# SiftScience/kafka-assigner

Hardware: NVIDIA H100
Metric: partition-replica assignments/sec (higher is better)
Workload: dtype int32

## Files before the change

kafka_assigner_b200/csrc/kassign.cu:

```cuda
#include "kassign_stage.cuh"
#include "kassign_order.cuh"
#include "kassign_json.cuh"
#include "kassign_score.cuh"
#include "kassign_waves.cuh"
#include "kassign_waves_json.cuh"

#include <algorithm>
#include <climits>
#include <cmath>
#include <cstdio>
#include <cstdlib>
#include <cstring>
#include <map>
#include <new>
#include <string>
#include <unordered_map>
#include <vector>

#include "../../include/kassign.h"

namespace {

constexpr int KA_SM_COUNT_FALLBACK = 132;
constexpr size_t KA_SMEM_BUDGET = 200 * 1024;
constexpr uint32_t KA_LUT_SMEM_MAX_RANGE = 32768;
constexpr uint32_t KA_LUT_GLOBAL_MAX_RANGE = 1u << 25;

struct DevBuf {
    void* p = nullptr;
    size_t cap = 0;
    cudaError_t reserve(size_t bytes) {
        if (bytes <= cap) return cudaSuccess;
        if (p) cudaFree(p);
        p = nullptr;
        cap = 0;
        size_t want = bytes + bytes / 8 + 256;
        cudaError_t e = cudaMalloc(&p, want);
        if (e == cudaSuccess) cap = want;
        return e;
    }
    void release() {
        if (p) cudaFree(p);
        p = nullptr;
        cap = 0;
    }
    template <typename T> T* as() const { return reinterpret_cast<T*>(p); }
};

constexpr int KA_MAX_BLOCKS = 8;
constexpr int KA_MAX_CHAIN_BLOCKS = 8;
constexpr int KA_MAX_CHAIN_EVENTS = 64;
constexpr int KA_MAX_JSON_FRAGS = 256;
constexpr int KA_MAX_CANDIDATES = 128;
static_assert(KA_MAX_CANDIDATES <= KA_JSON_MAX_SEGS, "a fleet's documents are built in one segmented JSON pass");
constexpr int64_t KA_JSON_FRAG_ROWS = 1 << 18;

struct HostPinned {
    int err_topic;
    int spin_flag;
    int4 tstatus;
};

struct Plan {
    int a_blob_bytes;
    int a_warps, a_load_bytes, a_slab_bytes, a_cnt_bytes, a_load_kind;
    int a_levels;
    int lv_owner_bytes, lv_last_bytes, lv_p_bytes;
    size_t a_smem;
    int rec_kind, rec_bytes;
    int b_gctr;
    int b_ring_log2;
    int b_threads;
    size_t b_smem;
};

struct StageDesc {
    int topic_base = 0, T = 0;
    int64_t Q = 0;
    const int32_t* d_hash = nullptr;
    const int64_t* d_part_off = nullptr;
    const int64_t* d_rep_off = nullptr;
    int P = 0, RF = 0;
    const int32_t* d_cur = nullptr;
    int desired_rf = -1, S = 1, Pmax = 0;
// ... 19 lines not shown
    }
};

}

struct ka_ctx {
    int device = 0;
    int sm_count = KA_SM_COUNT_FALLBACK;
    cudaStream_t stream = nullptr;
    cudaStream_t aux = nullptr;
    cudaStream_t sb1 = nullptr;
    cudaStream_t sj = nullptr;
    KaBrokers br{};
    std::vector<int32_t> broker_id;
    DevBuf d_blob, d_glut, d_broker_id, d_ctr8;
    std::unordered_map<int32_t, std::vector<int32_t>> parked;
    int64_t launches = 0;
    DevBuf d_hash, d_part_off, d_rep_off, d_cur, d_out, d_out_len;
    RunScratch run;
    DevBuf d_json, d_names, d_name_off, d_part_id, d_json_rowlen, d_json_blocksum, d_json_state;
    DevBuf d_json_seg;
    DevBuf d_batch_tab, d_batch_ctr;
    RunScratch batch_run;
    DevBuf d_score_w, d_score_sum, d_score_brk, d_score_off;
    DevBuf d_wv_nrecv, d_wv_wave, d_wv_tmp, d_wv_rec, d_wv_cnt, d_wv_state, d_wv_log, d_wv_sum, d_wv_meta;
    DevBuf d_wv_send, d_wv_slog, d_wv_ssum;
    DevBuf d_wv_perm, d_wv_hist, d_wv_doc;
    DevBuf d_wv_part, d_wv_jump;
    DevBuf d_wv_back, d_wv_bscr;
    HostPinned* h_pin = nullptr;
    unsigned long long* h_frag = nullptr;
    cudaEvent_t ev[6] = {};
    cudaEvent_t ev_pipe[KA_MAX_BLOCKS][5] = {};
    cudaEvent_t ev_chain[KA_MAX_CHAIN_EVENTS][4] = {};
    cudaEvent_t ev_in = nullptr, ev_stage[KA_MAX_BLOCKS] = {}, ev_chain_in = nullptr, ev_b1[KA_MAX_CHAIN_EVENTS] = {};
    cudaEvent_t ev_json_in[KA_MAX_JSON_FRAGS] = {}, ev_json_scan[KA_MAX_JSON_FRAGS] = {}, ev_out_done = nullptr;
    bool timing = false;
    float last_ms[8] = {};
    bool ev_valid = false;
    int last_stages = 1;
    int chain_used = 0;
    bool slot_timed[2] = {false, false};
    int32_t order_plan[8] = {};
    int32_t stage_plan[8] = {};
    bool staged = false;
    StageDesc staged_block;
    int topic_base = 0;
    bool last_was_staged = false;
    cudaStream_t last_stream = nullptr;
    bool pending_status = false;
    ka_status last{};
};

namespace {

#define KA_CUDA(call)                                                                              \
    do {                                                                                           \
        cudaError_t _e = (call);                                                                   \
        if (_e != cudaSuccess) {                                                                   \
            std::fprintf(stderr, "[kassign] CUDA error %s at %s:%d: %s\n", cudaGetErrorName(_e), __FILE__, __LINE__, \
                         cudaGetErrorString(_e));                                                  \
            return KA_ERR_CUDA;                                                                    \
        }                                                                                          \
    } while (0)

int set_status(ka_status* st, int code, int topic = -1, int part = -1, int a = 0, int b = 0) {
    if (st) {
        st->code = code;
        st->topic_index = topic;
        st->partition = part;
        st->a = a;
        st->b = b;
    }
    return code;
}

int failed(ka_status* st, int rc) {
    if (st && st->code != rc) set_status(st, rc);
    return rc;
}

inline size_t align16(size_t v) { return (v + 15) & ~size_t(15); }

template <typename F>
void for_each_event(ka_ctx* c, F f) {
    const struct { cudaEvent_t* e; size_t n; bool timed; } pools[] = {
        {c->ev, sizeof(c->ev) / sizeof(cudaEvent_t), true},
        {&c->ev_pipe[0][0], sizeof(c->ev_pipe) / sizeof(cudaEvent_t), true},
        {&c->ev_chain[0][0], sizeof(c->ev_chain) / sizeof(cudaEvent_t), true},
        {&c->ev_in, 1, false},
        {c->ev_stage, KA_MAX_BLOCKS, false},
        {&c->ev_chain_in, 1, false},
        {c->ev_b1, KA_MAX_CHAIN_EVENTS, false},
        {c->ev_json_in, KA_MAX_JSON_FRAGS, false},
        {c->ev_json_scan, KA_MAX_JSON_FRAGS, false},
        {&c->ev_out_done, 1, false},
    };
    for (const auto& p : pools)
        for (size_t i = 0; i < p.n; ++i) f(p.e[i], p.timed);
}

int park_counters(ka_ctx* c) {
    if (c->br.N == 0 || !c->d_ctr8.p) return KA_OK;
    std::vector<int32_t> h((size_t)c->br.N * KA_MAX_SLOTS);
    KA_CUDA(cudaMemcpy(h.data(), c->d_ctr8.p, h.size() * 4, cudaMemcpyDeviceToHost));
    for (int i = 0; i < c->br.N; ++i) {
        const int32_t* row = h.data() + (size_t)i * KA_MAX_SLOTS;
        bool nz = false;
        for (int r = 0; r < KA_MAX_SLOTS; ++r) nz |= row[r] != 0;
        if (nz) c->parked[c->broker_id[i]] = std::vector<int32_t>(row, row + KA_MAX_SLOTS);
        else c->parked.erase(c->broker_id[i]);
    }
    return KA_OK;
}

int check_brokers(int N, const int32_t* broker_id, const int32_t* broker_rack) {
    if (N < 0 || (N > 0 && (!broker_id || !broker_rack))) return KA_ERR_BAD_ARG;
    if (N > 65535) return KA_ERR_LIMIT;
    for (int i = 0; i < N; ++i) {
        if (i > 0 && broker_id[i] <= broker_id[i - 1]) return KA_ERR_BAD_ARG;
        if (broker_rack[i] < 0 || broker_rack[i] >= 65535) return KA_ERR_BAD_ARG;
    }
    return KA_OK;
}

struct BrokerTable {
// ... 254 lines not shown
    return p;
}

int enq_stage(ka_ctx* c, cudaStream_t s, const StageDesc& d, cudaEvent_t a_done) {
    const Plan& pl = d.pl;
    RunScratch& r = c->run;
    if (d.T > 0) {
        KaSolveParams p = stage_params(d);
        p.br = c->br;
        p.out.rec = r.rec.as<unsigned char>() + (size_t)d.q0 * pl.rec_bytes;
        p.out.perm = pl.a_levels ? r.perm.as<uint16_t>() + d.q0 : nullptr;
        p.out.ntl = pl.a_levels ? r.ntl.as<int32_t>() + d.topic_base : nullptr;
        p.out.lend = pl.a_levels ? r.lend.as<uint32_t>() + d.q0 : nullptr;
        p.out.tstatus = r.tstatus.as<int4>();
        p.out.err_topic = r.flags.as<unsigned>();
        const int rc = launch_stage_plan<false>(c, s, p, pl, d.T, 0, 1 << c->br.lut_mode);
        if (rc != KA_OK) return rc;
    }
    if (c->timing) KA_CUDA(cudaEventRecord(a_done, s));
    if (pl.a_levels && d.T > 0) {
        int32_t* ntl = r.ntl.as<int32_t>() + d.topic_base;
        int32_t* loff = r.loff.as<int32_t>() + d.topic_base + d.blk;
        ka_level_scan_kernel<<<1, 1024, 0, s>>>(ntl, d.T, loff);
        KA_CUDA(cudaGetLastError());
        ka_level_fill_kernel<<<(d.T + 7) / 8, 256, 0, s>>>(ntl, loff, r.lend.as<uint32_t>() + d.q0, d.d_part_off, d.P, d.T, d.T, d.Q,
                                                            r.lvl_end.as<uint32_t>() + d.q0);
        KA_CUDA(cudaGetLastError());
        c->launches += 2;
    }
    return KA_OK;
}

template <int KIND, int MAXNT, bool CAND, bool GCTR, bool SINGLE, bool WARP1, bool FULL>
cudaError_t launch_order_t(cudaStream_t s, const KaOrderParams& o, const Plan& pl, int ncand) {
    auto kern = ka_order_levels_kernel<KIND, GCTR, MAXNT, SINGLE, WARP1, FULL, CAND>;
    cudaError_t e = allow_smem(kern, pl.b_smem);
    if (e != cudaSuccess) return e;
    kern<<<CAND ? ncand : 1, pl.b_threads, pl.b_smem, s>>>(o);
    return cudaGetLastError();
}

template <int KIND, int MAXNT, bool CAND = false>
cudaError_t launch_order(cudaStream_t s, const KaOrderParams& o, const Plan& pl, int* sel, int ncand = 0) {
    if constexpr (KIND > 1) {
        *sel = pl.b_gctr ? 4 : 0;
        return pl.b_gctr ? launch_order_t<KIND, MAXNT, false, true, false, false, false>(s, o, pl, ncand)
                         : launch_order_t<KIND, MAXNT, false, false, false, false, false>(s, o, pl, ncand);
    } else {
        const bool warp1 = pl.b_threads == 32;
        const bool single = !warp1 && o.uniform_width != 0 && o.uniform_width <= (uint32_t)pl.b_threads;
        const bool full = single && o.uniform_width == (uint32_t)pl.b_threads;
        *sel = (pl.b_gctr ? 4 : 0) | (warp1 ? 1 : (full ? 3 : (single ? 2 : 0)));
        switch (*sel) {
            case 0: return launch_order_t<KIND, MAXNT, CAND, false, false, false, false>(s, o, pl, ncand);
            case 1: return launch_order_t<KIND, MAXNT, CAND, false, false, true, false>(s, o, pl, ncand);
            case 2: return launch_order_t<KIND, MAXNT, CAND, false, true, false, false>(s, o, pl, ncand);
            case 3: return launch_order_t<KIND, MAXNT, CAND, false, true, false, true>(s, o, pl, ncand);
            case 4: return launch_order_t<KIND, MAXNT, CAND, true, false, false, false>(s, o, pl, ncand);
            case 5: return launch_order_t<KIND, MAXNT, CAND, true, false, true, false>(s, o, pl, ncand);
            case 6: return launch_order_t<KIND, MAXNT, CAND, true, true, false, false>(s, o, pl, ncand);
            default: return launch_order_t<KIND, MAXNT, CAND, true, true, false, true>(s, o, pl, ncand);
        }
    }
}

void note_order(ka_ctx* c, const Plan& pl, int sel, int ncand) {
    int32_t* r = c->order_plan;
    r[0] = pl.rec_kind;
    r[1] = pl.a_levels;
    r[2] = pl.b_threads;
    r[3] = pl.b_ring_log2;
    r[4] = (sel >> 2) & 1;
    r[5] = sel & 3;
    r[6]++;
    r[7] = ncand;
}

int chain_subblocks(const StageDesc& d, int blocks_in_solve) {
    if (d.d_part_off || d.pl.rec_kind != 3 || d.T < 2) return 1;
    int n = std::max(1, 8 / std::max(1, blocks_in_solve));
    n = std::min(n, std::max(1, d.T / 128));
    if (const char* e = std::getenv("KA_CHAIN_SUBBLOCKS")) n = std::max(1, std::min(std::atoi(e), d.T));
    return std::min(n, KA_MAX_CHAIN_BLOCKS);
}

struct SolveCall {
    const int32_t* h_hash = nullptr;
    const int32_t* h_cur = nullptr;
    const int64_t* h_part_off = nullptr;
    const int64_t* h_rep_off = nullptr;
    const int32_t* h_part_id = nullptr;
    int32_t* d_part_id = nullptr;
    int32_t* d_out = nullptr;
    int32_t* d_out_len = nullptr;
    int32_t* h_out = nullptr;
    int32_t* h_out_len = nullptr;
    bool json = false;
    bool stream_out = false;
    int out_copies = 0;
    int json_blocks = 0;
    int chains = 0;

    SolveCall(int32_t* out, int32_t* out_len) : d_out(out), d_out_len(out_len) {}
};

SolveCall host_call(ka_ctx* c, const int32_t* topic_hash, const int64_t* part_off, const int64_t* rep_off, const int32_t* cur_broker,
                    int32_t* out_len, int32_t* out_broker, const int32_t* part_id = nullptr) {
    SolveCall io(c->d_out.as<int32_t>(), c->d_out_len.as<int32_t>());
    io.h_hash = topic_hash;
    io.h_part_off = part_off;
    io.h_rep_off = rep_off;
    io.h_cur = cur_broker;
    io.h_part_id = part_id;
    io.d_part_id = part_id ? c->d_part_id.as<int32_t>() : nullptr;
    io.h_out = out_broker;
    io.h_out_len = out_len;
    return io;
}

struct SubBlock { int t0, t1; int64_t r0, rq; };

SubBlock sub_block(const StageDesc& d, int j, int nsub) {
    SubBlock b;
    b.t0 = (int)((int64_t)d.T * j / nsub);
    b.t1 = (int)((int64_t)d.T * (j + 1) / nsub);
    b.r0 = d.d_part_off ? 0 : (int64_t)b.t0 * d.P;
    b.rq = d.d_part_off ? d.Q : (int64_t)(b.t1 - b.t0) * d.P;
    return b;
}

KaJsonParams json_params(ka_ctx* c, const int32_t* out, const int32_t* out_len, int S, int T, const int64_t* part_off,
                         const int32_t* part_id, int64_t row0, int64_t rows, unsigned long long cap) {
    KaJsonParams p{};
    p.Q = (uint32_t)rows;
// ... 69 lines not shown
        f.r0 = b.r0 + r;
        f.rq = std::min(step, b.rq - r);
        const int rc = enq_json_rows(c, s_done, io, d, f, first && r == 0, last && r + step >= b.rq);
        if (rc != KA_OK) return rc;
        r += step;
    } while (r < b.rq);
    return KA_OK;
}

int enq_copy_out(cudaStream_t s, const SolveCall& io, int S, int64_t r0, int64_t rows) {
    KA_CUDA(cudaMemcpyAsync(io.h_out + r0 * S, io.d_out + r0 * S, (size_t)rows * S * 4, cudaMemcpyDeviceToHost, s));
    if (io.h_out_len) KA_CUDA(cudaMemcpyAsync(io.h_out_len + r0, io.d_out_len + r0, (size_t)rows * 4, cudaMemcpyDeviceToHost, s));
    return KA_OK;
}

KaOrderParams order_params(ka_ctx* c, const StageDesc& d, const SubBlock& b) {
    const Plan& pl = d.pl;
    KaOrderParams o{};
    o.N = c->br.N;
    o.S = d.S;
    o.uniform_width = pl.a_levels ? 0u : (uint32_t)d.P;
    o.chunk_end = pl.a_levels ? c->run.lvl_end.as<uint32_t>() + d.q0 : nullptr;
    o.ctr8 = c->d_ctr8.as<int32_t>();
    o.ring_log2 = pl.b_ring_log2;
    const int32_t* loff = pl.a_levels ? c->run.loff.as<int32_t>() + d.topic_base + d.blk : nullptr;
    o.Q = (uint32_t)b.rq;
    o.rec = c->run.rec.as<unsigned char>() + (size_t)(d.q0 + b.r0) * pl.rec_bytes;
    o.pos_base = (uint32_t)b.r0;
    o.chunk_lo_ptr = loff ? loff + b.t0 : nullptr;
    o.chunk_hi_ptr = loff ? loff + b.t1 : nullptr;
    return o;
}

int enq_slot_chain(ka_ctx* c, cudaStream_t s, const StageDesc& d, int slot, int j, int nsub) {
    const SubBlock b = sub_block(d, j, nsub);
    if (b.rq <= 0 || c->br.N <= 0) return KA_OK;
    const KaOrderParams o = order_params(c, d, b);
    int sel = 0;
    KA_CUDA((slot == 0 ? launch_order<0, 1024>(s, o, d.pl, &sel) : launch_order<1, 1024>(s, o, d.pl, &sel)));
    note_order(c, d.pl, sel, 0);
    c->launches++;
    return KA_OK;
}

int enq_emit_block(ka_ctx* c, cudaStream_t s, const StageDesc& d, int j, int nsub, int32_t* d_out, int32_t* d_out_len) {
    const Plan& pl = d.pl;
    const SubBlock b = sub_block(d, j, nsub);
    if (b.rq <= 0 || c->br.N <= 0) return KA_OK;
    ka_emit3_kernel<<<(unsigned)((b.rq + 255) / 256), 256, 0, s>>>(
        reinterpret_cast<const uint4*>(c->run.rec.as<unsigned char>() + (size_t)(d.q0 + b.r0) * pl.rec_bytes),
        pl.a_levels ? c->run.perm.as<uint16_t>() + d.q0 + b.r0 : nullptr, d.d_part_off, b.t1 - b.t0, d.P, c->d_broker_id.as<int32_t>(),
        (uint32_t)b.rq, d.S, d_out + (size_t)b.r0 * d.S, d_out_len ? d_out_len + b.r0 : nullptr, c->d_ctr8.as<int32_t>());
    KA_CUDA(cudaGetLastError());
    c->launches++;
    return KA_OK;
}

int enq_order_emit(ka_ctx* c, cudaStream_t s, const StageDesc& d, SolveCall& io, int blocks_in_solve) {
    const int S = d.S;
    const Plan& pl = d.pl;
    if (d.Q <= 0 || c->br.N <= 0) return io.json && d.d_part_off && d.Q == 0 ? enq_json(c, s, io, d, sub_block(d, 0, 1), true, true) : KA_OK;
    int32_t* d_out = io.d_out + d.q0 * S;
    int32_t* d_out_len = io.d_out_len ? io.d_out_len + d.q0 : nullptr;
    if (pl.rec_kind != 3) {
        const SubBlock b = sub_block(d, 0, 1);
        KaOrderParams o = order_params(c, d, b);
        o.broker_id = c->d_broker_id.as<int32_t>();
        o.out = d_out;
        o.out_len = d_out_len;
        int sel = 0;
        KA_CUDA((pl.rec_kind == 4 ? launch_order<4, 512>(s, o, pl, &sel) : launch_order<8, 256>(s, o, pl, &sel)));
        note_order(c, pl, sel, 0);
        c->launches++;
        if (io.json) return enq_json(c, s, io, d, b, d.blk == 0, d.blk == blocks_in_solve - 1);
        return KA_OK;
    }
    const int nsub = chain_subblocks(d, blocks_in_solve);
    cudaStream_t s1 = c->sb1;
    for (int j = 0; j < nsub; ++j) {
        const int e = io.chains % KA_MAX_CHAIN_EVENTS;
        if (c->timing) KA_CUDA(cudaEventRecord(c->ev_chain[e][0], s1));
        int rc = enq_slot_chain(c, s1, d, 0, j, nsub);
        if (rc != KA_OK) return rc;
        if (c->timing) KA_CUDA(cudaEventRecord(c->ev_chain[e][1], s1));
        KA_CUDA(cudaEventRecord(c->ev_b1[e], s1));
        KA_CUDA(cudaStreamWaitEvent(s, c->ev_b1[e], 0));
        if (c->timing) KA_CUDA(cudaEventRecord(c->ev_chain[e][2], s));
        if ((rc = enq_slot_chain(c, s, d, 1, j, nsub)) != KA_OK) return rc;
        if ((rc = enq_emit_block(c, s, d, j, nsub, d_out, d_out_len)) != KA_OK) return rc;
        if (c->timing) KA_CUDA(cudaEventRecord(c->ev_chain[e][3], s));
        const SubBlock b = sub_block(d, j, nsub);
        if (io.stream_out) {
            cudaStream_t so = s;
            if (io.out_copies < KA_MAX_CHAIN_EVENTS) {
                KA_CUDA(cudaEventRecord(c->ev_json_in[io.out_copies], s));
                KA_CUDA(cudaStreamWaitEvent(c->sj, c->ev_json_in[io.out_copies], 0));
                io.out_copies++;
                so = c->sj;
            }
            if ((rc = enq_copy_out(so, io, S, d.q0 + b.r0, b.rq)) != KA_OK) return rc;
        }
        if (io.json) {
            if ((rc = enq_json(c, s, io, d, b, d.blk == 0 && j == 0, d.blk == blocks_in_solve - 1 && j == nsub - 1)) != KA_OK)
                return rc;
        }
        c->chain_used = std::min(++io.chains, KA_MAX_CHAIN_EVENTS);
    }
    return KA_OK;
}

int chain_fork(ka_ctx* c, cudaStream_t s) {
    KA_CUDA(cudaEventRecord(c->ev_chain_in, s));
    KA_CUDA(cudaStreamWaitEvent(c->sb1, c->ev_chain_in, 0));
    return KA_OK;
}

int enq_solve_end(ka_ctx* c, cudaStream_t s) {
    KA_CUDA(cudaMemcpyAsync(&c->h_pin->err_topic, c->run.flags.p, 2 * sizeof(int), cudaMemcpyDeviceToHost, s));
    if (c->timing) {
        KA_CUDA(cudaEventRecord(c->ev[5], s));
        c->ev_valid = true;
    }
    return KA_OK;
}

int pipeline_stages(int T, int64_t Q) {
    int k = Q >= 262144 ? std::min(4, T / 2048) : 1;
    if (const char* e = std::getenv("KA_PIPELINE_STAGES")) k = std::atoi(e);
    return std::max(1, std::min(k, std::min(KA_MAX_BLOCKS, std::max(T, 1))));
}

int enq_inputs(cudaStream_t s, const SolveCall& io, const StageDesc& d, int64_t ncur) {
    auto h2d = [&](const void* dst, const void* src, size_t bytes) {
        return cudaMemcpyAsync(const_cast<void*>(dst), src, bytes, cudaMemcpyHostToDevice, s);
    };
    if (io.h_hash && d.T > 0) KA_CUDA(h2d(d.d_hash, io.h_hash + d.topic_base, (size_t)d.T * 4));
    if (io.h_part_off && d.T > 0) KA_CUDA(h2d(d.d_part_off, io.h_part_off, (size_t)(d.T + 1) * 8));
    if (io.h_rep_off && d.Q > 0) KA_CUDA(h2d(d.d_rep_off, io.h_rep_off, (size_t)(d.Q + 1) * 8));
    if (io.h_part_id && d.Q > 0) KA_CUDA(h2d(io.d_part_id, io.h_part_id, (size_t)d.Q * 4));
    if (io.h_cur && ncur > 0) KA_CUDA(h2d(d.d_cur, io.h_cur + d.q0 * d.RF, (size_t)ncur * 4));
    return KA_OK;
}

int run_solve(ka_ctx* c, cudaStream_t s, const Shape& sh, SolveCall& io, ka_status* st) {
    c->staged = false;
    c->last_was_staged = false;
    reset_plans(c);
    const bool ragged = sh.d_part_off != nullptr;
    const int T = sh.T;
    const int K = ragged ? 1 : pipeline_stages(T, (int64_t)T * sh.P);
    const bool host_io = (io.h_cur != nullptr || io.h_out != nullptr) && K >= 3;
    const int wsum = host_io ? 2 * (K - 1) : K;
    auto bound = [&](int k) { return k <= 0 ? 0 : (k >= K ? T : (int)((int64_t)T * (host_io ? 2 * k - 1 : k) / wsum)); };
    StageDesc ds[KA_MAX_BLOCKS];
    int rc;
    for (int k = 0; k < K; ++k)
        if ((rc = describe_block(sh, bound(k), bound(k + 1), k, c->br.N, c->br.blob_bytes, ds[k], st)) != KA_OK) return rc;
    if ((rc = reserve_scratch(c, ds, K)) != KA_OK) return rc;
    c->last_stages = K;
    if (c->timing) KA_CUDA(cudaEventRecord(c->ev[0], s));
    if (K == 1) {
        const StageDesc& d = ds[0];
        if ((rc = enq_inputs(s, io, d, ragged ? sh.R : d.Q * d.RF)) != KA_OK) return rc;
        if ((rc = reset_flags(c, s)) != KA_OK) return rc;
        if (c->timing) KA_CUDA(cudaEventRecord(c->ev[1], s));
        if ((rc = enq_stage(c, s, d, c->ev[2])) != KA_OK) return rc;
        if (c->timing) KA_CUDA(cudaEventRecord(c->ev[3], s));
        if ((rc = chain_fork(c, s)) != KA_OK) return rc;
        if ((rc = enq_order_emit(c, s, d, io, 1)) != KA_OK) return rc;
        if (c->timing) KA_CUDA(cudaEventRecord(c->ev[4], s));
        if (io.h_out && d.Q > 0 && c->br.N > 0 && (rc = enq_copy_out(s, io, d.S, 0, d.Q)) != KA_OK) return rc;
    } else {
        cudaStream_t aux = c->aux;
        io.stream_out = io.h_out && ds[0].pl.rec_kind == 3 && !io.json;
        KA_CUDA(cudaEventRecord(c->ev_in, s));
        if (io.stream_out) KA_CUDA(cudaStreamWaitEvent(c->sj, c->ev_in, 0));
        KA_CUDA(cudaStreamWaitEvent(aux, c->ev_in, 0));
        if ((rc = reset_flags(c, aux)) != KA_OK) return rc;
        for (int k = 0; k < K; ++k) {
            const StageDesc& d = ds[k];
            if ((rc = enq_inputs(aux, io, d, d.Q * d.RF)) != KA_OK) return rc;
            if (c->timing) KA_CUDA(cudaEventRecord(c->ev_pipe[k][0], aux));
            if ((rc = enq_stage(c, aux, d, c->ev_pipe[k][1])) != KA_OK) return rc;
            if (c->timing) KA_CUDA(cudaEventRecord(c->ev_pipe[k][2], aux));
            KA_CUDA(cudaEventRecord(c->ev_stage[k], aux));
            KA_CUDA(cudaStreamWaitEvent(s, c->ev_stage[k], 0));
            KA_CUDA(cudaStreamWaitEvent(c->sb1, c->ev_stage[k], 0));
            if (k == 0) KA_CUDA(cudaStreamWaitEvent(c->sb1, c->ev_in, 0));
            if (c->timing) KA_CUDA(cudaEventRecord(c->ev_pipe[k][3], s));
            if ((rc = enq_order_emit(c, s, d, io, K)) != KA_OK) return rc;
            if (c->timing) KA_CUDA(cudaEventRecord(c->ev_pipe[k][4], s));
            if (io.h_out && !io.stream_out && d.Q > 0 && c->br.N > 0 && (rc = enq_copy_out(s, io, d.S, d.q0, d.Q)) != KA_OK) return rc;
        }
        if (io.stream_out) {
            KA_CUDA(cudaEventRecord(c->ev_out_done, c->sj));
            KA_CUDA(cudaStreamWaitEvent(s, c->ev_out_done, 0));
        }
    }
    return enq_solve_end(c, s);
}

ka_status topic_status(int t, const int4& ts, const int32_t* part_id, const int64_t* part_off) {
    ka_status r;
    set_status(&r, ts.x, t, ts.y >= 0 && part_id && part_off ? part_id[part_off[t] + ts.y] : ts.y, ts.z, ts.w);
    return r;
}

int finish_status(ka_ctx* c, cudaStream_t s, ka_status* st, const int32_t* part_id = nullptr, const int64_t* part_off = nullptr) {
    KA_CUDA(cudaStreamSynchronize(s));
    c->pending_status = false;
    ka_status r{};
    set_status(&r, KA_OK);
    if (c->h_pin->err_topic != -1) {
        const int t = c->h_pin->err_topic;
        KA_CUDA(cudaMemcpy(&c->h_pin->tstatus, c->run.tstatus.as<int4>() + t, sizeof(int4), cudaMemcpyDeviceToHost));
        r = topic_status(t, c->h_pin->tstatus, part_id, part_off);
        r.topic_index += c->last_was_staged ? c->topic_base : 0;
    }
    if (c->timing && c->ev_valid) {
        for (int i = 0; i < 8; ++i) c->last_ms[i] = 0.f;
        cudaEventElapsedTime(&c->last_ms[5], c->ev[0], c->ev[5]);
        if (c->last_stages <= 1) {
            cudaEventElapsedTime(&c->last_ms[3], c->ev[0], c->ev[1]);
            cudaEventElapsedTime(&c->last_ms[0], c->ev[1], c->ev[2]);
            cudaEventElapsedTime(&c->last_ms[1], c->ev[2], c->ev[3]);
            cudaEventElapsedTime(&c->last_ms[7], c->ev[3], c->ev[4]);
// ... 575 lines not shown
        (rc = reserve_scratch(c, &d, 1)) != KA_OK)
        return rc;
    c->last_stages = 1;
    if (c->timing) { cudaEventRecord(c->ev[0], s); cudaEventRecord(c->ev[1], s); }
    if ((rc = reset_flags(c, s)) != KA_OK || (rc = enq_stage(c, s, d, c->ev[2])) != KA_OK) return rc;
    if (c->timing) cudaEventRecord(c->ev[3], s);
    c->staged = true;
    return KA_OK;
}

static int enter_staged(ka_ctx* c, bool slot_chains, ka_status* st) {
    set_status(st, KA_OK);
    if (!c) return set_status(st, KA_ERR_NO_DEVICE);
    const int rc = enter(c, false);
    if (rc != KA_OK) return failed(st, rc);
    if (!c->staged || (slot_chains && c->staged_block.pl.rec_kind != 3)) return set_status(st, KA_ERR_BAD_ARG);
    return KA_OK;
}

static int end_staged(ka_ctx* c, cudaStream_t s, ka_status* st) {
    if (c->timing) cudaEventRecord(c->ev[4], s);
    const int rc = enq_solve_end(c, s);
    if (rc != KA_OK) return failed(st, rc);
    c->staged = false;
    c->last_was_staged = true;
    return finish(c, s, st, false);
}

int32_t ka_order_device(ka_ctx* c, int32_t* d_out_len, int32_t* d_out_broker, void* stream, ka_status* st) {
    int rc = enter_staged(c, false, st);
    if (rc != KA_OK) return rc;
    cudaStream_t s = (cudaStream_t)stream;
    SolveCall io(d_out_broker, d_out_len);
    if ((rc = chain_fork(c, s)) != KA_OK || (rc = enq_order_emit(c, s, c->staged_block, io, 1)) != KA_OK) return failed(st, rc);
    return end_staged(c, s, st);
}

int32_t ka_staged_slot_chains(ka_ctx* c) {
    if (!c || !c->staged) return 0;
    return c->staged_block.pl.rec_kind == 3 ? 2 : 0;
}

int32_t ka_order_slot_device(ka_ctx* c, int32_t slot, void* stream) {
    int rc = enter_staged(c, true, nullptr);
    if (rc != KA_OK) return rc;
    if (slot < 0 || slot > 1) return KA_ERR_BAD_ARG;
    const StageDesc& d = c->staged_block;
    cudaStream_t s = (cudaStream_t)stream;
    const int nsub = chain_subblocks(d, 1);
    if (c->timing) cudaEventRecord(c->ev_chain[slot][0], s);
    for (int j = 0; j < nsub; ++j)
        if ((rc = enq_slot_chain(c, s, d, slot, j, nsub)) != KA_OK) return rc;
    if (c->timing) cudaEventRecord(c->ev_chain[slot][1], s);
    c->slot_timed[slot] = c->timing;
    return KA_OK;
}

int32_t ka_emit_device(ka_ctx* c, int32_t* d_out_len, int32_t* d_out_broker, void* stream, ka_status* st) {
    int rc = enter_staged(c, true, st);
    if (rc != KA_OK) return rc;
    if (!d_out_broker) return set_status(st, KA_ERR_BAD_ARG);
    cudaStream_t s = (cudaStream_t)stream;
    if ((rc = enq_emit_block(c, s, c->staged_block, 0, 1, d_out_broker, d_out_len)) != KA_OK) return failed(st, rc);
    return end_staged(c, s, st);
}

static int copy_counter_column(ka_ctx* c, int slot, int32_t* d_col, const int32_t* d_src, cudaStream_t s) {
// ... 1066 lines not shown
```

kafka_assigner_b200/csrc/kassign_order.cuh:

```cuda
#pragma once
#include "kassign_common.cuh"

__global__ void __launch_bounds__(1024) ka_level_scan_kernel(const int32_t* __restrict__ ntl, int T, int32_t* __restrict__ loff) {
    const int total = ka_cta_scan(ntl, loff, T, 0);
    if (threadIdx.x == 0) loff[T] = total;
}

__global__ void __launch_bounds__(256) ka_level_fill_kernel(const int32_t* __restrict__ ntl, const int32_t* __restrict__ loff,
                                                            const uint32_t* __restrict__ lend, const int64_t* __restrict__ part_off, int P,
                                                            int T, int U, int64_t rows, uint32_t* __restrict__ lvl_end) {
    const int lane = threadIdx.x & 31;
    const int u = (blockIdx.x * blockDim.x + threadIdx.x) >> 5;
    if (u >= U) return;
    const int k = u / T, t = u - k * T;
    const int64_t g0 = (int64_t)k * rows + (part_off ? part_off[t] : (int64_t)t * P);
    const int d = ntl[u], o = loff[u];
    for (int l = lane; l < d; l += 32) lvl_end[o + l] = (uint32_t)g0 + lend[g0 + l];
}

struct KaOrderParams {
    uint32_t Q;
    int N;
    int S;
    const void* rec;
    uint32_t uniform_width;
    const uint32_t* chunk_end;
    const int32_t* chunk_lo_ptr;
    const int32_t* chunk_hi_ptr;
    uint32_t pos_base;
    int32_t* ctr8;
    const int32_t* broker_id;
    int32_t* out;
    int32_t* out_len;
    int ring_log2;
    const KaCandidate* cand;
    int cand_t0, cand_t1;
};

#define KA_RING_STAGES 8

__device__ __forceinline__ void ka_mbar_arrive(uint64_t* bar) {
    asm volatile("mbarrier.arrive.shared::cta.b64 _, [%0];" ::"r"(ka_smem_u32(bar)) : "memory");
}
__device__ __forceinline__ void ka_named_bar_sync(uint32_t id, uint32_t nthreads) {
    asm volatile("bar.sync %0, %1;" ::"r"(id), "r"(nthreads) : "memory");
}

template <bool GCTR> struct KaCtr;
template <> struct KaCtr<false> {
    typedef uint32_t H;
    template <int CW> static __device__ __forceinline__ H row(uint32_t sbase, int32_t*, uint32_t a) { return sbase + (CW == 4 ? a : a * 2u); }
    static __device__ __forceinline__ int4 ld4(H h, int off) {
        int4 v;
        asm volatile("ld.volatile.shared.v4.s32 {%0,%1,%2,%3}, [%4];" : "=r"(v.x), "=r"(v.y), "=r"(v.z), "=r"(v.w) : "r"(h + off));
        return v;
    }
    static __device__ __forceinline__ void st(H h, int off, int v) { asm volatile("st.volatile.shared.s32 [%0], %1;" ::"r"(h + off), "r"(v) : "memory"); }
    static __device__ __forceinline__ H col(uint32_t sbase, int32_t*, uint32_t a, int) { return sbase + a; }
    static __device__ __forceinline__ int ld1(H h) {
        int v;
        asm volatile("ld.volatile.shared.s32 %0, [%1];" : "=r"(v) : "r"(h));
        return v;
    }
    static __device__ __forceinline__ void st1(H h, int v) { asm volatile("st.volatile.shared.s32 [%0], %1;" ::"r"(h), "r"(v) : "memory"); }
};
template <> struct KaCtr<true> {
    typedef char* H;
    template <int CW> static __device__ __forceinline__ H row(uint32_t, int32_t* g, uint32_t a) { return reinterpret_cast<char*>(g) + (size_t)a * 2u; }
    static __device__ __forceinline__ int4 ld4(H h, int off) {
        int4 v;
        asm volatile("ld.volatile.global.v4.s32 {%0,%1,%2,%3}, [%4];" : "=r"(v.x), "=r"(v.y), "=r"(v.z), "=r"(v.w) : "l"(h + off));
        return v;
    }
    static __device__ __forceinline__ void st(H h, int off, int v) { asm volatile("st.volatile.global.s32 [%0], %1;" ::"l"(h + off), "r"(v) : "memory"); }
    static __device__ __forceinline__ H col(uint32_t, int32_t* g, uint32_t a, int slot) { return reinterpret_cast<char*>(g) + (size_t)a * 8u + slot * 4; }
    static __device__ __forceinline__ int ld1(H h) {
        int v;
        asm volatile("ld.volatile.global.s32 %0, [%1];" : "=r"(v) : "l"(h));
        return v;
// ... 33 lines not shown
    constexpr int RB = RS == 3 ? 16 : 32;
    constexpr int NS = KA_RING_STAGES;
    typedef KaCtr<GCTR> C;
    extern __shared__ __align__(128) unsigned char ka_osmem[];
    const uint32_t tid = threadIdx.x, lane = tid & 31;
    unsigned char* ring = ka_osmem;
    uint64_t* full = reinterpret_cast<uint64_t*>(ka_osmem + ((size_t)NS << p.ring_log2) * RB);
    volatile uint32_t* pin = reinterpret_cast<volatile uint32_t*>(full + 2 * NS);
    int* ctr = reinterpret_cast<int*>(ka_osmem + ((size_t)NS << p.ring_log2) * RB + 256);
    static_assert(!CAND || KIND <= 1, "batched solves order rows of <= 3 replicas");
    const KaCandidate* const cd = CAND ? p.cand + blockIdx.x : nullptr;
    if (CAND && (cd->br.N <= 0 || p.pos_base >= cd->Q)) return;
    if (tid == 0) {
        const void* const rec = CAND ? (const void*)(cd->out.rec + ((size_t)cd->row0 + p.pos_base) * RB) : p.rec;
        int32_t* const c8 = CAND ? cd->ctr8 : p.ctr8;
        pin[0] = CAND ? min(p.Q, cd->Q - p.pos_base) : p.Q;
        pin[1] = blockDim.x; pin[2] = (uint32_t)p.ring_log2; pin[3] = p.uniform_width;
        pin[4] = (uint32_t)reinterpret_cast<uintptr_t>(rec); pin[5] = (uint32_t)(reinterpret_cast<uintptr_t>(rec) >> 32);
        pin[6] = (uint32_t)reinterpret_cast<uintptr_t>(c8); pin[7] = (uint32_t)(reinterpret_cast<uintptr_t>(c8) >> 32);
        if (CAND) pin[8] = (uint32_t)cd->br.N;
    }
    __syncthreads();
    const uint32_t Q = pin[0], NT = pin[1];
    const int LG = (int)pin[2];
    const uint32_t w = pin[3];
    uint4* const orec = reinterpret_cast<uint4*>((uintptr_t)pin[4] | ((uintptr_t)pin[5] << 32));
    int32_t* const ctr8 = reinterpret_cast<int32_t*>((uintptr_t)pin[6] | ((uintptr_t)pin[7] << 32));
    const uint32_t G = 1u << LG;

    if (tid == 0) {
        for (int i = 0; i < NS; ++i) ka_mbar_init(&full[i], 1);
        ka_fence_mbar_init();
    }
    if (!GCTR)
        for (uint32_t i = tid; i < (uint32_t)(CAND ? (int)pin[8] : p.N) * CW; i += blockDim.x)
            ctr[i] = ctr8[(i / CW) * KA_MAX_SLOTS + (KIND <= 1 ? KIND : (int)(i % CW))];
    if (KIND <= 1 && tid == 0) {
        const int N = CAND ? (int)pin[8] : p.N;
        if (GCTR) ctr8[(size_t)N * KA_MAX_SLOTS + KIND] = 0x7FFFFFFF; else ctr[N] = 0x7FFFFFFF;
    }
    for (uint32_t i = tid; i < (uint32_t)NS * G * (RB / 16); i += blockDim.x) reinterpret_cast<uint4*>(ring)[i] = make_uint4(0, 0, 0, 0);
    ka_fence_proxy_async();
    __syncthreads();

    const uint32_t nstages_all = (Q + G - 1) >> LG;
    auto issue_stage = [&](uint32_t j) {
        const uint32_t slot = j & (NS - 1);
        const uint32_t bytes = min(G, Q - (j << LG)) * RB;
        ka_mbar_expect_tx(&full[slot], bytes);
        ka_tma_bulk_g2s(ring + (size_t)slot * G * RB, reinterpret_cast<const unsigned char*>(CAND ? (const void*)orec : p.rec) + (size_t)j * G * RB,
                        bytes, &full[slot]);
    };
    if (tid == 0)
        for (uint32_t j = 0; j < min(nstages_all, (uint32_t)NS); ++j) issue_stage(j);

    const uint32_t rmask = (uint32_t)NS * G - 1u;
    const uint32_t ring_s = ka_smem_u32(ring);
    uint32_t landed = 0;
    uint32_t released = 0;
    const int chunk_lo = w ? 0 : (CAND ? cd->loff[min(p.cand_t0, cd->T)] : *p.chunk_lo_ptr);
    const int nchunk = w ? 0 : (CAND ? cd->loff[min(p.cand_t1, cd->T)] : *p.chunk_hi_ptr) - chunk_lo;
    const uint32_t* const cend = p.chunk_end + chunk_lo;
    const uint32_t pos_base = CAND ? cd->pos0 + p.pos_base : p.pos_base;
    int wbase = 0;
    uint32_t wcur = Q, wnxt = Q;
    if (!w) {
        wcur = (int)lane < nchunk ? cend[lane] - pos_base : Q;
        wnxt = 32 + (int)lane < nchunk ? cend[32 + lane] - pos_base : Q;
    }
    uint32_t lvl_hi = w;
    int c = 0;
    auto next_end = [&](uint32_t cur_end) -> uint32_t {
        if (w) {
            if (cur_end == lvl_hi) lvl_hi += w;
            return min(min(cur_end + NT, lvl_hi), Q);
        }
        ++c;
        if (c >= nchunk) return Q;
        if (c >= wbase + 32) {
            wcur = wnxt;
            wbase += 32;
            const int i = wbase + 32 + (int)lane;
            wnxt = i < nchunk ? cend[i] - pos_base : Q;
        }
        return __shfl_sync(KA_FULL, wcur, c - wbase);
    };
    auto read_rec = [&](uint32_t pos, uint4& a, uint4& b) {
// ... 218 lines not shown
#pragma unroll
                    for (int v = 0; v < RS; ++v) cv[i][v] = 0;
                }
            }
            const uint32_t nstart = end;
            const uint32_t nend = next_end(end);
            if (nend > limit) cross_to(end, nend);
            read_rec(nstart + tid, nb0, nb1);
            int perm[RS];
#pragma unroll
            for (int i = 0; i < RS; ++i) perm[i] = i;
            if (len > 0) ka_order_generic<RS>(cv, len, meta, perm);
#pragma unroll
            for (int r = 0; r < RS; ++r) {
                if (r < len) {
                    uint32_t ba = 0;
                    int cc = 0;
#pragma unroll
                    for (int q = 0; q < RS; ++q)
                        if (perm[r] == q) { ba = av[q]; cc = cv[q][r]; }
                    C::st(C::template row<CW>(cbase, ctr8, ba), r * 4, cc + 1);
                    if (r < p.S) p.out[(size_t)orow * p.S + r] = __ldg(&p.broker_id[ba >> 4]);
                } else if (active && r < p.S) {
                    p.out[(size_t)orow * p.S + r] = -1;
                }
            }
            if (active && p.out_len) p.out_len[orow] = len;
            if (NT == 32) __syncwarp(); else __syncthreads();
            start = nstart; end = nend;
            ra0 = nb0; ra1 = nb1;
        }
    }

    if (!GCTR) {
        if (NT == 32) __syncwarp(); else __syncthreads();
        for (uint32_t i = tid; i < (uint32_t)(CAND ? (int)pin[8] : p.N) * CW; i += NT) ctr8[(i / CW) * KA_MAX_SLOTS + (KIND <= 1 ? KIND : (int)(i % CW))] = ctr[i];
    }
}

__device__ __forceinline__ void ka_emit3(const uint4* __restrict__ rec, const uint16_t* __restrict__ perm,
                                         const int64_t* __restrict__ part_off, int T, int P, const int32_t* __restrict__ broker_id,
                                         uint32_t Q, int S, int32_t* __restrict__ out, int32_t* __restrict__ out_len,
                                         int32_t* __restrict__ ctr8, uint32_t base = 0) {
    const uint32_t pos = blockIdx.x * blockDim.x + threadIdx.x;
    if (pos >= Q) return;
    const uint4 r = rec[pos];
    const int len = (int)(r.w & 3u);
    uint32_t row = pos;
    if (perm) {
        int64_t g0;
        if (part_off) {
            int lo = 0, hi = T;
            while (hi - lo > 1) {
                const int mid = (lo + hi) >> 1;
                if (part_off[mid] <= (int64_t)(base + pos)) lo = mid; else hi = mid;
            }
            g0 = part_off[lo] - base;
        } else {
            g0 = (int64_t)(pos / (uint32_t)P) * P;
        }
        row = (uint32_t)g0 + perm[pos];
    }
    int32_t* o = out + (size_t)row * S;
    o[0] = len > 0 ? __ldg(broker_id + (r.x >> 2)) : -1;
    if (S > 1) o[1] = len > 1 ? __ldg(broker_id + (r.y >> 2)) : -1;
    if (S > 2) o[2] = len > 2 ? __ldg(broker_id + (r.z >> 2)) : -1;
// ... 24 lines not shown
```

Baseline: 2.921 billion.

## Overlap chained order kernels with PDL and move emits to a side stream

Order-level kernels in a chain now launch with programmatic stream serialization. Each kernel issues its TMA prologue before griddepcontrol.wait and signals dependents before writing back counters, so consecutive sub-block kernels overlap their setup. Emit, copy-out and JSON work for each sub-block moves to a separate stream and is joined at the end. The change also allows more chain sub-blocks for large blocks, skips ring zeroing in the FULL variant, and splits staging from ordering into two loops so all stages are enqueued first. Risks: PDL ordering must keep the counter hand-off correct, and more sub-blocks add more launches and events.

```diff
diff --git a/kafka_assigner_b200/csrc/kassign.cu b/kafka_assigner_b200/csrc/kassign.cu
--- a/kafka_assigner_b200/csrc/kassign.cu
+++ b/kafka_assigner_b200/csrc/kassign.cu
@@ -48,8 +48,8 @@
 };
 
 constexpr int KA_MAX_BLOCKS = 8;
-constexpr int KA_MAX_CHAIN_BLOCKS = 8;
-constexpr int KA_MAX_CHAIN_EVENTS = 64;
+constexpr int KA_MAX_CHAIN_BLOCKS = 16;
+constexpr int KA_MAX_CHAIN_EVENTS = KA_MAX_BLOCKS * KA_MAX_CHAIN_BLOCKS;
 constexpr int KA_MAX_JSON_FRAGS = 256;
 constexpr int KA_MAX_CANDIDATES = 128;
 static_assert(KA_MAX_CANDIDATES <= KA_JSON_MAX_SEGS, "a fleet's documents are built in one segmented JSON pass");
@@ -135,8 +135,9 @@
     unsigned long long* h_frag = nullptr;
     cudaEvent_t ev[6] = {};
     cudaEvent_t ev_pipe[KA_MAX_BLOCKS][5] = {};
-    cudaEvent_t ev_chain[KA_MAX_CHAIN_EVENTS][4] = {};
+    cudaEvent_t ev_chain[KA_MAX_BLOCKS][4] = {};
     cudaEvent_t ev_in = nullptr, ev_stage[KA_MAX_BLOCKS] = {}, ev_chain_in = nullptr, ev_b1[KA_MAX_CHAIN_EVENTS] = {};
+    cudaEvent_t ev_b2[KA_MAX_CHAIN_EVENTS] = {}, ev_emit_done = nullptr;
     cudaEvent_t ev_json_in[KA_MAX_JSON_FRAGS] = {}, ev_json_scan[KA_MAX_JSON_FRAGS] = {}, ev_out_done = nullptr;
     bool timing = false;
     float last_ms[8] = {};
@@ -195,6 +196,8 @@
         {c->ev_stage, KA_MAX_BLOCKS, false},
         {&c->ev_chain_in, 1, false},
         {c->ev_b1, KA_MAX_CHAIN_EVENTS, false},
+        {c->ev_b2, KA_MAX_CHAIN_EVENTS, false},
+        {&c->ev_emit_done, 1, false},
         {c->ev_json_in, KA_MAX_JSON_FRAGS, false},
         {c->ev_json_scan, KA_MAX_JSON_FRAGS, false},
         {&c->ev_out_done, 1, false},
@@ -515,34 +518,43 @@
 }
 
 template <int KIND, int MAXNT, bool CAND, bool GCTR, bool SINGLE, bool WARP1, bool FULL>
-cudaError_t launch_order_t(cudaStream_t s, const KaOrderParams& o, const Plan& pl, int ncand) {
+cudaError_t launch_order_t(cudaStream_t s, const KaOrderParams& o, const Plan& pl, int ncand, bool behind) {
     auto kern = ka_order_levels_kernel<KIND, GCTR, MAXNT, SINGLE, WARP1, FULL, CAND>;
     cudaError_t e = allow_smem(kern, pl.b_smem);
     if (e != cudaSuccess) return e;
-    kern<<<CAND ? ncand : 1, pl.b_threads, pl.b_smem, s>>>(o);
-    return cudaGetLastError();
+    cudaLaunchAttribute attr{};
+    attr.id = cudaLaunchAttributeProgrammaticStreamSerialization;
+    attr.val.programmaticStreamSerializationAllowed = 1;
+    cudaLaunchConfig_t cfg{};
+    cfg.gridDim = dim3(CAND ? ncand : 1);
+    cfg.blockDim = dim3(pl.b_threads);
+    cfg.dynamicSmemBytes = pl.b_smem;
+    cfg.stream = s;
+    cfg.attrs = &attr;
+    cfg.numAttrs = behind ? 1 : 0;
+    return cudaLaunchKernelEx(&cfg, kern, o);
 }
 
 template <int KIND, int MAXNT, bool CAND = false>
-cudaError_t launch_order(cudaStream_t s, const KaOrderParams& o, const Plan& pl, int* sel, int ncand = 0) {
+cudaError_t launch_order(cudaStream_t s, const KaOrderParams& o, const Plan& pl, int* sel, int ncand = 0, bool behind = false) {
     if constexpr (KIND > 1) {
         *sel = pl.b_gctr ? 4 : 0;
-        return pl.b_gctr ? launch_order_t<KIND, MAXNT, false, true, false, false, false>(s, o, pl, ncand)
-                         : launch_order_t<KIND, MAXNT, false, false, false, false, false>(s, o, pl, ncand);
+        return pl.b_gctr ? launch_order_t<KIND, MAXNT, false, true, false, false, false>(s, o, pl, ncand, behind)
+                         : launch_order_t<KIND, MAXNT, false, false, false, false, false>(s, o, pl, ncand, behind);
     } else {
         const bool warp1 = pl.b_threads == 32;
         const bool single = !warp1 && o.uniform_width != 0 && o.uniform_width <= (uint32_t)pl.b_threads;
         const bool full = single && o.uniform_width == (uint32_t)pl.b_threads;
         *sel = (pl.b_gctr ? 4 : 0) | (warp1 ? 1 : (full ? 3 : (single ? 2 : 0)));
         switch (*sel) {
-            case 0: return launch_order_t<KIND, MAXNT, CAND, false, false, false, false>(s, o, pl, ncand);
-            case 1: return launch_order_t<KIND, MAXNT, CAND, false, false, true, false>(s, o, pl, ncand);
-            case 2: return launch_order_t<KIND, MAXNT, CAND, false, true, false, false>(s, o, pl, ncand);
-            case 3: return launch_order_t<KIND, MAXNT, CAND, false, true, false, true>(s, o, pl, ncand);
-            case 4: return launch_order_t<KIND, MAXNT, CAND, true, false, false, false>(s, o, pl, ncand);
-            case 5: return launch_order_t<KIND, MAXNT, CAND, true, false, true, false>(s, o, pl, ncand);
-            case 6: return launch_order_t<KIND, MAXNT, CAND, true, true, false, false>(s, o, pl, ncand);
-            default: return launch_order_t<KIND, MAXNT, CAND, true, true, false, true>(s, o, pl, ncand);
+            case 0: return launch_order_t<KIND, MAXNT, CAND, false, false, false, false>(s, o, pl, ncand, behind);
+            case 1: return launch_order_t<KIND, MAXNT, CAND, false, false, true, false>(s, o, pl, ncand, behind);
+            case 2: return launch_order_t<KIND, MAXNT, CAND, false, true, false, false>(s, o, pl, ncand, behind);
+            case 3: return launch_order_t<KIND, MAXNT, CAND, false, true, false, true>(s, o, pl, ncand, behind);
+            case 4: return launch_order_t<KIND, MAXNT, CAND, true, false, false, false>(s, o, pl, ncand, behind);
+            case 5: return launch_order_t<KIND, MAXNT, CAND, true, false, true, false>(s, o, pl, ncand, behind);
+            case 6: return launch_order_t<KIND, MAXNT, CAND, true, true, false, false>(s, o, pl, ncand, behind);
+            default: return launch_order_t<KIND, MAXNT, CAND, true, true, false, true>(s, o, pl, ncand, behind);
         }
     }
 }
@@ -559,10 +571,14 @@
     r[7] = ncand;
 }
 
-int chain_subblocks(const StageDesc& d, int blocks_in_solve) {
+constexpr int KA_CHAIN_SUB_TOPICS = 512;
+constexpr int KA_CHAIN_LARGE_BLOCK = 1024;
+
+int chain_subblocks(const StageDesc& d, int blocks_in_solve, bool overlapped = false) {
     if (d.d_part_off || d.pl.rec_kind != 3 || d.T < 2) return 1;
     int n = std::max(1, 8 / std::max(1, blocks_in_solve));
     n = std::min(n, std::max(1, d.T / 128));
+    if (overlapped && d.T >= KA_CHAIN_LARGE_BLOCK) n = std::max(n, d.T / KA_CHAIN_SUB_TOPICS);
     if (const char* e = std::getenv("KA_CHAIN_SUBBLOCKS")) n = std::max(1, std::min(std::atoi(e), d.T));
     return std::min(n, KA_MAX_CHAIN_BLOCKS);
 }
@@ -580,9 +596,9 @@
     int32_t* h_out_len = nullptr;
     bool json = false;
     bool stream_out = false;
-    int out_copies = 0;
     int json_blocks = 0;
     int chains = 0;
+    bool emits = false;
 
     SolveCall(int32_t* out, int32_t* out_len) : d_out(out), d_out_len(out_len) {}
 };
@@ -718,12 +734,12 @@
     return o;
 }
 
-int enq_slot_chain(ka_ctx* c, cudaStream_t s, const StageDesc& d, int slot, int j, int nsub) {
+int enq_slot_chain(ka_ctx* c, cudaStream_t s, const StageDesc& d, int slot, int j, int nsub, bool behind = false) {
     const SubBlock b = sub_block(d, j, nsub);
     if (b.rq <= 0 || c->br.N <= 0) return KA_OK;
     const KaOrderParams o = order_params(c, d, b);
     int sel = 0;
-    KA_CUDA((slot == 0 ? launch_order<0, 1024>(s, o, d.pl, &sel) : launch_order<1, 1024>(s, o, d.pl, &sel)));
+    KA_CUDA((slot == 0 ? launch_order<0, 1024>(s, o, d.pl, &sel, 0, behind) : launch_order<1, 1024>(s, o, d.pl, &sel, 0, behind)));
     note_order(c, d.pl, sel, 0);
     c->launches++;
     return KA_OK;
@@ -761,37 +777,40 @@
         if (io.json) return enq_json(c, s, io, d, b, d.blk == 0, d.blk == blocks_in_solve - 1);
         return KA_OK;
     }
-    const int nsub = chain_subblocks(d, blocks_in_solve);
-    cudaStream_t s1 = c->sb1;
+    const int nsub = chain_subblocks(d, blocks_in_solve, true);
+    const int e = c->chain_used;
+    if (e >= KA_MAX_BLOCKS || io.chains + nsub > KA_MAX_CHAIN_EVENTS) return KA_ERR_LIMIT;
+    cudaStream_t s1 = c->sb1, se = c->sj;
+    if (c->timing) KA_CUDA(cudaEventRecord(c->ev_chain[e][0], s1));
     for (int j = 0; j < nsub; ++j) {
-        const int e = io.chains % KA_MAX_CHAIN_EVENTS;
-        if (c->timing) KA_CUDA(cudaEventRecord(c->ev_chain[e][0], s1));
-        int rc = enq_slot_chain(c, s1, d, 0, j, nsub);
+        const int k = io.chains + j;
+        int rc = enq_slot_chain(c, s1, d, 0, j, nsub, true);
         if (rc != KA_OK) return rc;
-        if (c->timing) KA_CUDA(cudaEventRecord(c->ev_chain[e][1], s1));
-        KA_CUDA(cudaEventRecord(c->ev_b1[e], s1));
-        KA_CUDA(cudaStreamWaitEvent(s, c->ev_b1[e], 0));
-        if (c->timing) KA_CUDA(cudaEventRecord(c->ev_chain[e][2], s));
-        if ((rc = enq_slot_chain(c, s, d, 1, j, nsub)) != KA_OK) return rc;
-        if ((rc = enq_emit_block(c, s, d, j, nsub, d_out, d_out_len)) != KA_OK) return rc;
-        if (c->timing) KA_CUDA(cudaEventRecord(c->ev_chain[e][3], s));
+        KA_CUDA(cudaEventRecord(c->ev_b1[k], s1));
+        KA_CUDA(cudaStreamWaitEvent(s, c->ev_b1[k], 0));
+        if (c->timing && j == 0) KA_CUDA(cudaEventRecord(c->ev_chain[e][2], s));
+        if ((rc = enq_slot_chain(c, s, d, 1, j, nsub, true)) != KA_OK) return rc;
+        KA_CUDA(cudaEventRecord(c->ev_b2[k], s));
+        KA_CUDA(cudaStreamWaitEvent(se, c->ev_b2[k], 0));
+        if ((rc = enq_emit_block(c, se, d, j, nsub, d_out, d_out_len)) != KA_OK) return rc;
+        if (j == nsub - 1) {
+            if (c->timing) KA_CUDA(cudaEventRecord(c->ev_chain[e][3], se));
+            KA_CUDA(cudaEventRecord(c->ev_emit_done, se));
+            io.emits = true;
+        }
         const SubBlock b = sub_block(d, j, nsub);
-        if (io.stream_out) {
-            cudaStream_t so = s;
-            if (io.out_copies < KA_MAX_CHAIN_EVENTS) {
-                KA_CUDA(cudaEventRecord(c->ev_json_in[io.out_copies], s));
-                KA_CUDA(cudaStreamWaitEvent(c->sj, c->ev_json_in[io.out_copies], 0));
-                io.out_copies++;
-                so = c->sj;
-            }
-            if ((rc = enq_copy_out(so, io, S, d.q0 + b.r0, b.rq)) != KA_OK) return rc;
-        }
-        if (io.json) {
-            if ((rc = enq_json(c, s, io, d, b, d.blk == 0 && j == 0, d.blk == blocks_in_solve - 1 && j == nsub - 1)) != KA_OK)
-                return rc;
-        }
-        c->chain_used = std::min(++io.chains, KA_MAX_CHAIN_EVENTS);
-    }
+        if (io.stream_out && (rc = enq_copy_out(se, io, S, d.q0 + b.r0, b.rq)) != KA_OK) return rc;
+        if (io.json && (rc = enq_json(c, se, io, d, b, d.blk == 0 && j == 0, d.blk == blocks_in_solve - 1 && j == nsub - 1)) != KA_OK)
+            return rc;
+    }
+    if (c->timing) KA_CUDA(cudaEventRecord(c->ev_chain[e][1], s1));
+    io.chains += nsub;
+    c->chain_used = e + 1;
+    return KA_OK;
+}
+
+int join_emits(ka_ctx* c, cudaStream_t s, const SolveCall& io) {
+    if (io.emits) KA_CUDA(cudaStreamWaitEvent(s, c->ev_emit_done, 0));
     return KA_OK;
 }
 
@@ -853,7 +872,7 @@
         if ((rc = enq_stage(c, s, d, c->ev[2])) != KA_OK) return rc;
         if (c->timing) KA_CUDA(cudaEventRecord(c->ev[3], s));
         if ((rc = chain_fork(c, s)) != KA_OK) return rc;
-        if ((rc = enq_order_emit(c, s, d, io, 1)) != KA_OK) return rc;
+        if ((rc = enq_order_emit(c, s, d, io, 1)) != KA_OK || (rc = join_emits(c, s, io)) != KA_OK) return rc;
         if (c->timing) KA_CUDA(cudaEventRecord(c->ev[4], s));
         if (io.h_out && d.Q > 0 && c->br.N > 0 && (rc = enq_copy_out(s, io, d.S, 0, d.Q)) != KA_OK) return rc;
     } else {
@@ -870,6 +889,9 @@
             if ((rc = enq_stage(c, aux, d, c->ev_pipe[k][1])) != KA_OK) return rc;
             if (c->timing) KA_CUDA(cudaEventRecord(c->ev_pipe[k][2], aux));
             KA_CUDA(cudaEventRecord(c->ev_stage[k], aux));
+        }
+        for (int k = 0; k < K; ++k) {
+            const StageDesc& d = ds[k];
             KA_CUDA(cudaStreamWaitEvent(s, c->ev_stage[k], 0));
             KA_CUDA(cudaStreamWaitEvent(c->sb1, c->ev_stage[k], 0));
             if (k == 0) KA_CUDA(cudaStreamWaitEvent(c->sb1, c->ev_in, 0));
@@ -878,6 +900,7 @@
             if (c->timing) KA_CUDA(cudaEventRecord(c->ev_pipe[k][4], s));
             if (io.h_out && !io.stream_out && d.Q > 0 && c->br.N > 0 && (rc = enq_copy_out(s, io, d.S, d.q0, d.Q)) != KA_OK) return rc;
         }
+        if ((rc = join_emits(c, s, io)) != KA_OK) return rc;
         if (io.stream_out) {
             KA_CUDA(cudaEventRecord(c->ev_out_done, c->sj));
             KA_CUDA(cudaStreamWaitEvent(s, c->ev_out_done, 0));
@@ -1519,7 +1542,9 @@
     if (rc != KA_OK) return rc;
     cudaStream_t s = (cudaStream_t)stream;
     SolveCall io(d_out_broker, d_out_len);
-    if ((rc = chain_fork(c, s)) != KA_OK || (rc = enq_order_emit(c, s, c->staged_block, io, 1)) != KA_OK) return failed(st, rc);
+    if ((rc = chain_fork(c, s)) != KA_OK || (rc = enq_order_emit(c, s, c->staged_block, io, 1)) != KA_OK ||
+        (rc = join_emits(c, s, io)) != KA_OK)
+        return failed(st, rc);
     return end_staged(c, s, st);
 }
 
diff --git a/kafka_assigner_b200/csrc/kassign_order.cuh b/kafka_assigner_b200/csrc/kassign_order.cuh
--- a/kafka_assigner_b200/csrc/kassign_order.cuh
+++ b/kafka_assigner_b200/csrc/kassign_order.cuh
@@ -45,6 +45,8 @@
 __device__ __forceinline__ void ka_named_bar_sync(uint32_t id, uint32_t nthreads) {
     asm volatile("bar.sync %0, %1;" ::"r"(id), "r"(nthreads) : "memory");
 }
+__device__ __forceinline__ void ka_grid_dependency_wait() { asm volatile("griddepcontrol.wait;" ::: "memory"); }
+__device__ __forceinline__ void ka_launch_dependents() { asm volatile("griddepcontrol.launch_dependents;" ::: "memory"); }
 
 template <bool GCTR> struct KaCtr;
 template <> struct KaCtr<false> {
@@ -144,14 +146,8 @@
         for (int i = 0; i < NS; ++i) ka_mbar_init(&full[i], 1);
         ka_fence_mbar_init();
     }
-    if (!GCTR)
-        for (uint32_t i = tid; i < (uint32_t)(CAND ? (int)pin[8] : p.N) * CW; i += blockDim.x)
-            ctr[i] = ctr8[(i / CW) * KA_MAX_SLOTS + (KIND <= 1 ? KIND : (int)(i % CW))];
-    if (KIND <= 1 && tid == 0) {
-        const int N = CAND ? (int)pin[8] : p.N;
-        if (GCTR) ctr8[(size_t)N * KA_MAX_SLOTS + KIND] = 0x7FFFFFFF; else ctr[N] = 0x7FFFFFFF;
-    }
-    for (uint32_t i = tid; i < (uint32_t)NS * G * (RB / 16); i += blockDim.x) reinterpret_cast<uint4*>(ring)[i] = make_uint4(0, 0, 0, 0);
+    if (!FULL)
+        for (uint32_t i = tid; i < (uint32_t)NS * G * (RB / 16); i += blockDim.x) reinterpret_cast<uint4*>(ring)[i] = make_uint4(0, 0, 0, 0);
     ka_fence_proxy_async();
     __syncthreads();
 
@@ -165,6 +161,16 @@
     };
     if (tid == 0)
         for (uint32_t j = 0; j < min(nstages_all, (uint32_t)NS); ++j) issue_stage(j);
+
+    ka_grid_dependency_wait();
+    if (!GCTR)
+        for (uint32_t i = tid; i < (uint32_t)(CAND ? (int)pin[8] : p.N) * CW; i += blockDim.x)
+            ctr[i] = ctr8[(i / CW) * KA_MAX_SLOTS + (KIND <= 1 ? KIND : (int)(i % CW))];
+    if (KIND <= 1 && tid == 0) {
+        const int N = CAND ? (int)pin[8] : p.N;
+        if (GCTR) ctr8[(size_t)N * KA_MAX_SLOTS + KIND] = 0x7FFFFFFF; else ctr[N] = 0x7FFFFFFF;
+    }
+    __syncthreads();
 
     const uint32_t rmask = (uint32_t)NS * G - 1u;
     const uint32_t ring_s = ka_smem_u32(ring);
@@ -449,6 +455,7 @@
         }
     }
 
+    ka_launch_dependents();
     if (!GCTR) {
         if (NT == 32) __syncwarp(); else __syncthreads();
         for (uint32_t i = tid; i < (uint32_t)(CAND ? (int)pin[8] : p.N) * CW; i += NT) ctr8[(i / CW) * KA_MAX_SLOTS + (KIND <= 1 ? KIND : (int)(i % CW))] = ctr[i];
```

New measurement: 3.117 billion (median of 6 runs). 6.7% higher.
